# google-research/hyperbo

Measured on AMD Instinct MI355X. Metric: GP NLL+grad evals/sec at N=8192 D=16 fp64, higher is better.
Workload: dtype f64

## Files before the change

### hyperbo_amd/csrc/chol.hip

```cpp
#include "hbo_internal.h"
#include <type_traits>
#include <limits.h>
#include <string.h>

namespace {

#include "panel_dev.h"
#ifdef HBO_POTF2_TIMING
__device__ unsigned long long hbo_dbg_stamps[64];
__device__ unsigned long long hbo_dbg_wall[3 * 256];
__device__ unsigned long long hbo_dbg_trsm[3 * 128];
__device__ int hbo_dbg_trsm_panel = 36;
#define STAMP(i) do { if (threadIdx.x == 0) hbo_dbg_stamps[i] = __builtin_readcyclecounter(); } while (0)
#else
#define STAMP(i) do {} while (0)
#endif
#ifndef HBO_POTF2_WAVES
#define HBO_POTF2_WAVES 8
#endif
constexpr int POTF2_WAVES = HBO_POTF2_WAVES;
constexpr int POTF2_THREADS = 64 * POTF2_WAVES;
template <typename T>
__device__ __forceinline__ void potf2_body(const TaskDesc& t, int p, int* info_slot, unsigned char* smem) {
  typedef typename Mma<T>::acc_t acc_t;
// ... 71 lines not shown

  int nleaf = 8;
  {
    const int64_t rows = (int64_t)t.n - (int64_t)p * NB;
    if (rows < NB) nleaf = rows <= 0 ? 0 : (int)((rows + 15) / 16);
    for (int jb = nleaf + wave; jb < 8; jb += POTF2_WAVES)
#pragma unroll
      for (int r = 0; r < 4; ++r) {
        const int row = Mma<T>::crow(lane, r);
        gst(Wb + (int64_t)(jb * 16 + row) * ld + jb * 16 + l15, row == l15 ? (T)1 : (T)0);
      }
    if (tid < NB && tid >= nleaf * 16) sDinv[tid] = (T)1;
  }
  const bool lead_tile0 = nleaf > 0;
  acc_t tile0 = {0, 0, 0, 0};
  if (wave == 0 && lead_tile0) {
#pragma unroll
    for (int r = 0; r < 4; ++r) {
      const int row = Mma<T>::crow(lane, r);
      const int rr = row > l15 ? row : l15, cc = row > l15 ? l15 : row;
      tile0[r] = gld(Ab + (int64_t)rr * ld + cc);
    }
  }
  constexpr int NSH = POTF2_THREADS / 256;
  const int sh = __builtin_amdgcn_readfirstlane(tid >> 8);
  T vload[36 / NSH];
  auto load_issue = [&](auto share) {
    constexpr int SH = decltype(share)::value;
    int tile = 0;
#pragma unroll
    for (int I = 0; I < 8; ++I)
#pragma unroll
      for (int J = 0; J <= I; ++J, ++tile) {
        if (tile % NSH != SH) continue;
        if (tile == 0 && lead_tile0) { vload[0] = (T)0; continue; }
        int r = ei, c = ej;
        if (I == J && ej > ei) { r = ej; c = ei; }
        vload[tile / NSH] = gld(Ab + (int64_t)(I * 16 + r) * ld + J * 16 + c);
      }
  };
  auto load_commit = [&](auto share) {
    constexpr int SH = decltype(share)::value;
#pragma unroll
    for (int k = 0; k < 36 / NSH; ++k)
      if (!(k == 0 && SH == 0 && lead_tile0)) sT[(k * NSH + SH) * TILE_ELEMS + ei * TS + ej] = vload[k];
  };
  static_assert(NSH == 1 || NSH == 2, "one or two 256-thread groups");
  if (NSH == 1 || sh == 0) load_issue(std::integral_constant<int, 0>());
  else load_issue(std::integral_constant<int, NSH - 1>());
  if (wave == 0 && lead_tile0) factor_leaf(0, &tile0);
  if (NSH == 1 || sh == 0) load_commit(std::integral_constant<int, 0>());
  else load_commit(std::integral_constant<int, NSH - 1>());
  STAMP(1);
  __syncthreads();
  STAMP(2);
  for (int jb = 0; jb < nleaf; ++jb) {
    for (int R = jb + 1 + wave; R < nleaf; R += POTF2_WAVES) solve_tile(jb, R);
    __syncthreads();
    STAMP(3 + 3 * jb);
    if (jb == nleaf - 1) break;
    {
      const int m = nleaf - 1 - jb;
      const int ntiles = m * (m + 1) / 2;
      constexpr int NH = POTF2_WAVES == 8 ? 6 : POTF2_WAVES - 1;
      const int hw = POTF2_WAVES == 8 ? (wave < 4 ? wave : wave - 1) : wave;
      const int n0 = (ntiles - 1 > 4 * NH + 1) ? (ntiles - 1 - (4 * NH + 1)) / POTF2_WAVES : 0;
      const int nshared = ntiles - n0;
      auto tile_of = [&](int tix, int& I, int& J) {
        int ii = 0;
        while ((ii + 1) * (ii + 2) / 2 <= tix) ++ii;
        I = jb + 1 + ii; J = jb + 1 + tix - ii * (ii + 1) / 2;
      };
      if (wave == 0) {
        update_tile(jb, jb + 1, jb + 1);
        factor_leaf(jb + 1);
        STAMP(4 + 3 * jb);
        for (int tix = nshared; tix < ntiles; ++tix) { int I, J; tile_of(tix, I, J); update_tile(jb, I, J); }
      } else if (!(POTF2_WAVES == 8 && wave == 4)) {
        int tix = hw;
        for (; tix + NH < nshared; tix += 2 * NH) {
          int I0, J0, I1, J1;
          tile_of(tix, I0, J0); tile_of(tix + NH, I1, J1);
          update_tile2(jb, I0, J0, I1, J1);
        }
        if (tix < nshared) { int I, J; tile_of(tix, I, J); update_tile(jb, I, J); }
      }
    }
    __syncthreads();
    STAMP(5 + 3 * jb);
  }
  STAMP(30);

  auto store_share = [&](auto share) {
    constexpr int SH = decltype(share)::value;
    int tile = 0;
#pragma unroll
    for (int I = 0; I < 8; ++I)
#pragma unroll
      for (int J = 0; J <= I; ++J, ++tile) {
        if (tile % NSH != SH) continue;
        T v = sT[tile * TILE_ELEMS + ei * TS + ej];
        if (I == J && ej > ei) v = (T)0;
        gst(Ab + (int64_t)(I * 16 + ei) * ld + J * 16 + ej, v);
      }
  };
  if (NSH == 1 || sh == 0) store_share(std::integral_constant<int, 0>());
// ... 222 lines not shown
```

### hyperbo_amd/csrc/gram.hip

```cpp
#include "kernfun.h"

namespace {

template <typename T, bool PADDED, int KID>
__global__ __launch_bounds__(256) void gram_kernel(GramArgs g, const ModelDev* __restrict__ md) {
  typedef typename V16<T>::type vec_t;
  constexpr int VEC = 16 / sizeof(T);
  __shared__ T sA[DC * SXS];
  __shared__ T sB[DC * SXS];
  const int ti = blockIdx.y;
  const int tj = g.symmetric ? (int)((blockIdx.x + blockIdx.y) % gridDim.x) : (int)blockIdx.x;
  const T* x1; const T* x2; T* out; int64_t n1, n2, ldo; int64_t e1, e2;
  if (g.tasks) {
    const TaskDesc& t = g.tasks[blockIdx.z];
    md += (int64_t)blockIdx.z * g.model_stride;
    if ((int64_t)ti * GTR >= t.npad || tj >= t.nblk) return;
    x1 = x2 = static_cast<const T*>(t.F);
    out = static_cast<T*>(t.A);
    n1 = n2 = t.n; ldo = t.ld; e1 = e2 = t.npad;
  } else {
    x1 = static_cast<const T*>(g.x1); x2 = static_cast<const T*>(g.x2); out = static_cast<T*>(g.out);
    n1 = g.n1; n2 = g.n2; ldo = g.ldo; e1 = PADDED ? g.n1pad : g.n1; e2 = PADDED ? g.n2pad : g.n2;
  }
  const int64_t r0 = (int64_t)ti * GTR, c0 = (int64_t)tj * HBO_TILE;
  if (g.symmetric && c0 > r0 + GTR - 1) return;
  const int fdim = g.fdim;
  constexpr int kid = KID;
  constexpr bool is_dot = (kid == HBO_KERNEL_DOT);
  const int tid = threadIdx.x, tx = tid & 15, ty = tid >> 4;

  T acc[GRA][8];
#pragma unroll
  for (int a = 0; a < GRA; ++a)
#pragma unroll
    for (int b = 0; b < 8; ++b) acc[a][b] = (T)0;

  for (int d0 = 0; d0 < fdim; d0 += DC) {
    __syncthreads();
    stage_x<T, GRA>(sA, x1, n1, fdim, r0, d0, md->inv_ls, !is_dot, tid);
    stage_x<T, 8>(sB, x2, n2, fdim, c0, d0, md->inv_ls, !is_dot, tid);
    __syncthreads();
    const int dlim = (fdim - d0) < DC ? (fdim - d0) : DC;
    auto step = [&](int dd) {
      T av[GRA], bv[8];
#pragma unroll
      for (int a = 0; a < GRA; ++a) av[a] = sA[dd * SXS + ty + 16 * a];
#pragma unroll
      for (int q = 0; q < 8; ++q) bv[q] = sB[dd * SXS + 16 * VEC * (q / VEC) + VEC * tx + (q % VEC)];
      if (is_dot) {
#pragma unroll
        for (int a = 0; a < GRA; ++a)
#pragma unroll
          for (int q = 0; q < 8; ++q) acc[a][q] += av[a] * bv[q];
      } else {
#pragma unroll
        for (int a = 0; a < GRA; ++a)
#pragma unroll
          for (int q = 0; q < 8; ++q) { const T df = av[a] - bv[q]; acc[a][q] += df * df; }
      }
    };
    for (int dd = 0; dd < dlim; ++dd) step(dd);
  }

  const ExpCoef ec = hbo_exp_coef();
// ... 18 lines not shown
          vv[e] = kfun(kid, acc[a][qb * VEC + e], sv, inv_sigma2, bias2, ec);
#endif
        }
#ifdef HBO_GRAM_NOSTORE
        if (vv[0] == (T)123.456) gst(reinterpret_cast<vec_t*>(orow + 16 * VEC * qb), vv);
#else
        gst(reinterpret_cast<vec_t*>(orow + 16 * VEC * qb), vv);
#endif
      }
    }
    return;
  }
#pragma unroll
  for (int a = 0; a < GRA; ++a) {
    __builtin_amdgcn_sched_barrier(0);
    const int64_t row = r0 + ty + 16 * a;
    if (row >= e1) continue;
#pragma unroll
    for (int qb = 0; qb < 8 / VEC; ++qb) {
      const int64_t col0 = c0 + 16 * VEC * qb + VEC * tx;
      T vals[VEC];
#pragma unroll
      for (int e = 0; e < VEC; ++e) {
        const int64_t col = col0 + e;
        T v;
        if (row < n1 && col < n2) {
#ifdef HBO_GRAM_NOEXP
          v = acc[a][qb * VEC + e] * sv;
#else
          v = kfun(kid, acc[a][qb * VEC + e], sv, inv_sigma2, bias2, ec);
#endif
          if (g.symmetric && row == col) v += diag_add;
        } else {
          v = (g.symmetric && row == col) ? (T)1 : (T)0;
        }
        vals[e] = v;
      }
      if (PADDED) {
        vec_t vv;
#pragma unroll
        for (int e = 0; e < VEC; ++e) vv[e] = vals[e];
#ifdef HBO_GRAM_NOSTORE
        if (vv[0] == (T)123.456) gst(reinterpret_cast<vec_t*>(out + row * ldo + col0), vv);
#else
        gst(reinterpret_cast<vec_t*>(out + row * ldo + col0), vv);
#endif
      } else {
#pragma unroll
        for (int e = 0; e < VEC; ++e)
          if (col0 + e < e2) gst(out + row * ldo + col0 + e, vals[e]);
      }
    }
  }
}

typedef __bf16 gm_bf16x8 __attribute__((ext_vector_type(8)));
typedef float gm_f32x16 __attribute__((ext_vector_type(16)));
typedef unsigned short gm_u16x8 __attribute__((ext_vector_type(8)));
constexpr int GM_KC = 16;
constexpr int GM_ROWB = 2 * GM_KC + 16;
constexpr int GM_LPR = GM_KC / 4;
constexpr int GM_RPP = 256 / GM_LPR;
constexpr int GM_NQ = 256 / GM_RPP;
constexpr int GM_FS = HBO_TILE + 4;
constexpr float GM_RISK = 1e-6f / (32.f * 5.9604645e-8f);
constexpr unsigned GM_REDO = 0x7fc0d1e5u;
struct GmTile {
  const float* x1; const float* x2; const float* xc; float* out; const double* inv_ls;
  int64_t n1, n2, ldo, e1, e2, r0, c0;
  int fdim, nrow, ncol;
  bool symmetric, mirror, on_diag, interior;
  float sv, diag_add, risk_lim;
};
template <int KID>
__device__ __forceinline__ float gm_cov(float sv, float u) {
  if (KID == HBO_KERNEL_SE) return sv * __builtin_amdgcn_exp2f(u * (-0.5f * 1.44269504088896341f));
  const float r = __builtin_amdgcn_sqrtf((KID == HBO_KERNEL_MATERN32 ? 3.f : 5.f) * u);
  const float e = sv * __builtin_amdgcn_exp2f(r * -1.44269504088896341f);
  return KID == HBO_KERNEL_MATERN32 ? e * (1.f + r) : e * fmaf(r, fmaf(r, 1.f / 3.f, 1.f), 1.f);
}
template <int KID, bool DIRECT>
__device__ __forceinline__ bool gm_finish(const GmTile& t, const gm_f32x16 (&acc)[2][2], const float (*sN)[128]) {
  const int lane = threadIdx.x & 63, wave = threadIdx.x >> 6;
  const int wm = wave >> 1, wn = wave & 1, l32 = lane & 31, lh = lane >> 5;
  float risk = 0.f;
#pragma unroll
  for (int b = 0; b < 2; ++b) {
    const int rl = wm * 64 + b * 32 + l32;
    const float na = sN[0][rl];
    const int64_t gr = t.r0 + rl;
    float* orow = t.out + gr * t.ldo + t.c0;
#pragma unroll
    for (int a = 0; a < 2; ++a) {
      __builtin_amdgcn_sched_barrier(0);
#pragma unroll
      for (int j = 0; j < 4; ++j) {
        const int cl = wn * 64 + a * 32 + 8 * j + 4 * lh;
        const float4 nb4 = *reinterpret_cast<const float4*>(&sN[1][cl]);
        const float nbv[4] = {nb4.x, nb4.y, nb4.z, nb4.w};
        float val[4];
#pragma unroll
        for (int e = 0; e < 4; ++e) {
          const float s = acc[a][b][4 * j + e];
          const bool self = t.on_diag && rl == cl + e;
          val[e] = gm_cov<KID>(t.sv, self ? 0.f : (DIRECT ? s : fmaxf(na + nbv[e] - 2.f * s, 0.f)));
          if (!DIRECT) risk = fmaxf(risk, self ? 0.f : val[e] * (na + nbv[e]));
// ... 19 lines not shown
          }
        }
      }
    }
  }
  return risk > t.risk_lim;
}
template <int KID>
__device__ __forceinline__ void gm_direct_tile(const GmTile t, float* sF, const float (*sN)[128]) {
  const int tid = threadIdx.x, lane = tid & 63, wave = tid >> 6;
  const int wm = wave >> 1, wn = wave & 1, l32 = lane & 31, lh = lane >> 5;
  gm_f32x16 acc[2][2];
#pragma unroll
  for (int a = 0; a < 2; ++a)
#pragma unroll
    for (int b = 0; b < 2; ++b)
#pragma unroll
      for (int q = 0; q < 16; ++q) acc[a][b][q] = 0.f;
  for (int d0 = 0; d0 < t.fdim; d0 += GM_KC) {
    __syncthreads();
#pragma nounroll
    for (int i = tid; i < 2 * GM_KC * HBO_TILE; i += 256) {
      const int opq = i / (GM_KC * HBO_TILE), k = (i / HBO_TILE) % GM_KC, rr = i % HBO_TILE, d = d0 + k;
      const int64_t gr = (opq ? t.c0 : t.r0) + rr;
      float sx = 0.f;
      if (d < t.fdim && gr < (opq ? t.n2 : t.n1)) sx = ((opq ? t.x2 : t.x1)[gr * t.fdim + d] - t.xc[d]) * (float)t.inv_ls[d];
      sF[(opq * GM_KC + k) * GM_FS + rr] = sx;
    }
    __syncthreads();
#pragma nounroll
    for (int k = 0; k < GM_KC; ++k) {
      const float* fr = sF + k * GM_FS;
      const float* fc = sF + (GM_KC + k) * GM_FS;
#pragma unroll
      for (int b = 0; b < 2; ++b) {
        const float ra = fr[wm * 64 + b * 32 + l32];
#pragma unroll
        for (int a = 0; a < 2; ++a)
#pragma unroll
          for (int j = 0; j < 4; ++j) {
            const float4 cb = *reinterpret_cast<const float4*>(fc + wn * 64 + a * 32 + 8 * j + 4 * lh);
            const float cv[4] = {cb.x, cb.y, cb.z, cb.w};
#pragma unroll
            for (int e = 0; e < 4; ++e) { const float df = ra - cv[e]; acc[a][b][4 * j + e] = fmaf(df, df, acc[a][b][4 * j + e]); }
          }
      }
    }
  }
  gm_finish<KID, true>(t, acc, sN);
}
template <int KID>
__device__ __forceinline__ bool gm_make_tile(const GramArgs& g, const ModelDev*& md, GmTile& t) {
  const int ti = blockIdx.y;
  const int tj = g.symmetric ? (int)((blockIdx.x + blockIdx.y) % gridDim.x) : (int)blockIdx.x;
  if (g.tasks) {
    const TaskDesc& k = g.tasks[blockIdx.z];
    md += (int64_t)blockIdx.z * g.model_stride;
    if (ti >= k.nblk || tj >= k.nblk) return false;
    t.x1 = t.x2 = static_cast<const float*>(k.F);
    t.out = static_cast<float*>(k.A);
    t.n1 = t.n2 = k.n; t.ldo = k.ld; t.e1 = t.e2 = k.npad;
  } else {
    t.x1 = static_cast<const float*>(g.x1); t.x2 = static_cast<const float*>(g.x2); t.out = static_cast<float*>(g.out);
    t.n1 = g.n1; t.n2 = g.n2; t.ldo = g.ldo; t.e1 = g.padded ? g.n1pad : g.n1; t.e2 = g.padded ? g.n2pad : g.n2;
  }
  t.mirror = !g.tasks && !g.symmetric && t.x1 == t.x2 && t.n1 == t.n2;
  t.symmetric = g.symmetric;
  t.r0 = (int64_t)ti * HBO_TILE; t.c0 = (int64_t)tj * HBO_TILE;
  if ((g.symmetric || t.mirror) && tj > ti) return false;
  if (t.r0 >= t.e1 || t.c0 >= t.e2 || t.n1 <= 0) return false;
  t.fdim = g.fdim;
  t.xc = t.x1 + (t.r0 < t.n1 ? t.r0 : t.n1 - 1) * (int64_t)t.fdim;
  t.inv_ls = md->inv_ls;
  t.nrow = (int)min(t.n1 - t.r0, (int64_t)HBO_TILE); t.ncol = (int)min(t.n2 - t.c0, (int64_t)HBO_TILE);
  t.on_diag = (g.symmetric || t.mirror) && ti == tj;
  return true;
}
template <int KID>
__device__ __forceinline__ void gm_epilogue_fields(const ModelDev* md, GmTile& t) {
  t.interior = t.r0 + HBO_TILE <= t.n1 && t.c0 + HBO_TILE <= t.n2 && !t.on_diag && !t.mirror && (t.ldo & 3) == 0 &&
               (reinterpret_cast<unsigned long long>(t.out) & 15) == 0;
  t.sv = (float)md->sv; t.diag_add = (float)(md->noise + md->eps);
  constexpr float kappa = KID == HBO_KERNEL_SE ? 0.5f : (KID == HBO_KERNEL_MATERN32 ? 1.5f : 5.f / 6.f);
  t.risk_lim = (GM_RISK / kappa) * t.sv;
}
template <int KID>
__global__ __launch_bounds__(256, 3) void gram_mfma_kernel(GramArgs g, const ModelDev* __restrict__ md0) {
  __shared__ __attribute__((aligned(16))) unsigned char sP[2 * 3 * 128 * GM_ROWB];
  __shared__ float sN[2][128];
  GmTile t;
  const ModelDev* md = md0;
  if (!gm_make_tile<KID>(g, md, t)) return;
  const float* x1 = t.x1; const float* x2 = t.x2; const float* xc = t.xc; const double* inv_ls = t.inv_ls;
  const int64_t n1 = t.n1, n2 = t.n2, r0 = t.r0, c0 = t.c0;
  const int fdim = t.fdim;
  const int tid = threadIdx.x, lane = tid & 63, wave = tid >> 6;
  const int wm = wave >> 1, wn = wave & 1, l32 = lane & 31, lh = lane >> 5;

  const int sc4 = tid % GM_LPR, srow = tid / GM_LPR;
  const bool vec_ok = (fdim & 3) == 0 && ((reinterpret_cast<unsigned long long>(x1) | reinterpret_cast<unsigned long long>(x2)) & 15) == 0;
  auto load4 = [&](const float* xr, int d) -> float4 {
    if (vec_ok && d + 4 <= fdim) return *reinterpret_cast<const float4*>(xr + d);
    return make_float4(d < fdim ? xr[d] : 0.f, d + 1 < fdim ? xr[d + 1] : 0.f, d + 2 < fdim ? xr[d + 2] : 0.f, d + 3 < fdim ? xr[d + 3] : 0.f);
  };
  auto load_chunk = [&](int d0, float4 (&v)[GM_NQ]) {
    const int d = d0 + 4 * sc4;
#pragma unroll
// ... 409 lines not shown
```

### hyperbo_amd/csrc/hbo_internal.h

```cpp
#pragma once
#include <hip/hip_runtime.h>
#include <stdint.h>
#include "../../include/hbo.h"

#define HBO_GLOBAL __attribute__((address_space(1)))
template <typename V> __device__ __forceinline__ V gld(const V* p) { return *(const HBO_GLOBAL V*)(p); }
template <typename V> __device__ __forceinline__ void gst(V* p, V v) { *(HBO_GLOBAL V*)(p) = v; }

#define HBO_TILE 128
#define HBO_N_COUNTERS 4096
#define HBO_N_BULK_COUNTERS 1024
#define HBO_LEAF 16

struct TaskDesc {
  void* A;
  void* W;
  void* S;
  void* wscr;
  const void* X;
  const void* F;
  const void* Fm;
  const void* ysum;
  void* svec;
  void* dF;
// ... 112 lines not shown
  h = __builtin_bit_cast(unsigned short, hh); l = __builtin_bit_cast(unsigned short, ll);
}
__device__ __forceinline__ float hbo_h2_scale_for(float amax) {
  if (!(amax > 0.f) || !(amax < INFINITY)) return 1.f;
  int e;
  (void)frexpf(amax, &e);
  e = e < -40 ? -40 : e;
  return ldexpf(1.f, 14 - e);
}
__device__ __forceinline__ int yield_enter(int* tab) {
  const int tok = cu_token();
  __hip_atomic_fetch_add(tab + tok, 1, __ATOMIC_RELAXED, __HIP_MEMORY_SCOPE_AGENT);
  return tok;
}
__device__ __forceinline__ void yield_leave(int* tab, int tok) {
  __hip_atomic_fetch_add(tab + tok, -1, __ATOMIC_RELAXED, __HIP_MEMORY_SCOPE_AGENT);
}
__device__ __forceinline__ void tl_begin(unsigned long long* tl) {
#ifdef HBO_TIMELINE
  if (tl && threadIdx.x == 0) atomicMin(tl, (unsigned long long)wall_clock64());
#endif
}
__device__ __forceinline__ void tl_end(unsigned long long* tl) {
#ifdef HBO_TIMELINE
  if (tl && threadIdx.x == 0) atomicMax(tl + 1, (unsigned long long)wall_clock64());
#endif
}
#endif

static inline bool hbo_first_use_on_device(unsigned long long& seen) {
  int d = 0;
  if (hipGetDevice(&d) != hipSuccess || d < 0 || d >= 64) return true;
  if ((seen >> d) & 1ull) return false;
  seen |= 1ull << d;
  return true;
}

void launch_gemm(int dtype, const GemmArgs& a, dim3 grid, hipStream_t st);

void launch_potf2(int dtype, const TaskDesc* tasks, int ntasks, int p, int* info, hipStream_t st, int* yield_flag = nullptr,
                  unsigned long long* tl = nullptr);
void launch_trsm(int dtype, const TaskDesc* tasks, int ntasks, int p, int max_nblk, hipStream_t st, int* yield_tab = nullptr,
                 unsigned long long* tl = nullptr);
unsigned long long* tl_slot(const char* name, int p);
void launch_trtri_diag(int dtype, const TaskDesc* tasks, int ntasks, int p_lo, int p_hi, hipStream_t st);

struct GramArgs {
  const TaskDesc* tasks;
  const void* x1; const void* x2; void* out;
  int64_t n1, n2, ldo;
  int n1pad, n2pad;
  int fdim;
  int symmetric;
  int padded;
  int kernel_id;
  int direct_form;
  int mfma_min_f;
  int model_stride;
};
void launch_gram(int dtype, const GramArgs& a, const ModelDev* model, dim3 grid, hipStream_t st);
void launch_kdiag(int dtype, const void* f, int64_t n, int fdim, const ModelDev* model, void* out,
                  hipStream_t st);
void launch_dense_tanh(int dtype, const void* in, const void* w, const void* b, void* out, int64_t n,
                       int fin, int fout, hipStream_t st);
void launch_mean(int dtype, const void* fm, int64_t n, int fmean, const ModelDev* model, void* mu,
                 hipStream_t st);
void launch_aug_rows(int dtype, const TaskDesc* tasks, int ntasks, int max_npad, const ModelDev* md, hipStream_t st, int model_stride = 0);
void launch_poison(int dtype, const TaskDesc* tasks, int ntasks, int max_npad, hipStream_t st);
void launch_nll_reduce(int dtype, const TaskDesc* tasks, int ntasks, const int* info, double* out,
                       hipStream_t st);
void launch_wt_z(int dtype, const TaskDesc* tasks, int ntasks, int max_nblk, int aug_row, int out_col,
                 int out_ld, hipStream_t st, const void* xover = nullptr, void* oover = nullptr);
int grad_nacc(int kernel_id, int fdim);
void launch_grad_contract(int dtype, const TaskDesc* tasks, int ntasks, int max_nblk, const ModelDev* md,
                          int kernel_id, int fdim, int obj, double* partials, int64_t stride_task, hipStream_t st);
void launch_dmu(int dtype, const TaskDesc* tasks, int ntasks, int obj, hipStream_t st);
void launch_grad_finalize(int dtype, const TaskDesc* tasks, int ntasks, const ModelDev* md, int kernel_id,
                          int fdim, int obj, const double* partials, int64_t stride_task, double* out,
                          int out_stride, double* value_out, hipStream_t st, double* pre = nullptr, int max_nblk = 0);
constexpr int HBO_GRAD_PRE_ROWS = 32;
void launch_scale_dF(const TaskDesc* tasks, int ntasks, int64_t max_n, int fdim, hipStream_t st);
void launch_grad_feat(int dtype, const TaskDesc* tasks, int ntasks, int max_nblk, const ModelDev* md, int kernel_id,
                      int fdim, int obj, hipStream_t st);
void launch_grad_feat_mean(int dtype, const TaskDesc* tasks, int ntasks, int64_t max_n, const ModelDev* md,
                           int fdim, hipStream_t st);
void launch_dense_bwd(int dtype, const void* in, const void* out, const void* w, double* dout, double* din,
                      double* dW, double* db, int64_t n, int fin, int fout, hipStream_t st);
int small_eval_lds(int dtype);
void launch_small_eval(int dtype, const TaskDesc* tasks, int ntasks, const ModelDev* md, int kernel_id, int fdim, int* info,
                       double* nll_out, double* grad_out, int out_stride, int write_back, hipStream_t st, int tasks_per_model = 0);
struct MlpTaskDev {
  const void* x;
  void* acts[HBO_MAX_MLP_LAYERS];
  double* dF; double* dtmp;
  int64_t n;
  int64_t model;
};
void launch_mlp_forward_batch(int dtype, const MlpTaskDev* mt, int ntasks, int64_t max_n, int layer, const void* w, const void* b, int fin,
                              int fout, hipStream_t st, int model_weights = 0);
void launch_mlp_zero_dF_batch(const MlpTaskDev* mt, int ntasks, int64_t max_n, int flast, hipStream_t st);
void launch_dense_bwd_batch(int dtype, const MlpTaskDev* mt, int ntasks, int64_t max_n, int layer, int cur_is_dF, const void* w, double* dW,
                            double* db, int fin, int fout, int want_din, hipStream_t st);
void launch_kumar_forward(int dtype, const TaskDesc* tasks, int ntasks, int64_t max_n, const void* x, void* w, double* h, int64_t n, int D,
                          const ModelDev* md, hipStream_t st);
void launch_kumar_grad(int dtype, const TaskDesc* tasks, int ntasks, int max_nblk, const ModelDev* md, int kernel_id, int D, int obj,
                       double* partials, double* out, hipStream_t st);
void launch_kumar_chain_dx(int dtype, const void* xq, int64_t M, int D, const ModelDev* md, const double* gf, double* gx, hipStream_t st);
struct PostArgs {
  const void* Kxq; int64_t ldq; int npad; int n; int nblk;
  const void* alpha;
  const void* colsq;
// ... 109 lines not shown
```

### hyperbo_amd/csrc/objective.hip

```cpp
#include "api_internal.h"
#include <chrono>

extern "C" int hbo_nll(hbo_ctx* c, const hbo_model* m, hbo_dataset* ds, double* nll_sum, double* nll_per_task,
                       double* grad_sum) {
  return hbo_objective(c, m, ds, HBO_OBJ_NLL, nll_sum, nll_per_task, grad_sum);
}

int comm_allreduce_device(hbo_ctx* c, double* d_buf, int count, hipStream_t st);

int comm_abort(hbo_ctx* c);

static void enqueue_mlp_forward(hbo_ctx* c, const hbo_model* m, hbo_dataset* ds, int64_t max_n) {
  int fin = m->input_dim;
  for (int l = 0; l < m->n_layers; ++l) {
    launch_mlp_forward_batch(ds->dtype, ds->d_mlp, ds->ntasks, max_n, l, c->d_mlp_w[l], c->d_mlp_b[l], fin, m->features[l], c->stream);
    fin = m->features[l];
  }
}
static void enqueue_kumar_forward(hbo_ctx* c, const hbo_model* m, hbo_dataset* ds, int64_t max_n) {
  launch_kumar_forward(ds->dtype, ds->d_desc, ds->ntasks, max_n, nullptr, nullptr, nullptr, 0, m->input_dim, c->d_model, c->stream);
}
void enqueue_fused_forward(hbo_ctx* c, const hbo_model* m, hbo_dataset* ds, int64_t max_n, int out_stride, bool want_grad) {
  const bool kumar = is_kumar(m);
  if (needs_mlp(m)) { ProfScope ps(c, "features", 1); enqueue_mlp_forward(c, m, ds, max_n); }
// ... 146 lines not shown
    }
    if (!ds->d_mlp) HIPCHK(c, dev_alloc(c, (void**)&ds->d_mlp, sizeof(MlpTaskDev) * T));
    if (ds->h_mlp_dev.size() != (size_t)T || memcmp(ds->h_mlp_dev.data(), hm.data(), sizeof(MlpTaskDev) * T) != 0) {
      HIPCHK(c, hipStreamSynchronize(st));
      ds->h_mlp_dev = hm;
      HIPCHK(c, hipMemcpyAsync(ds->d_mlp, ds->h_mlp_dev.data(), sizeof(MlpTaskDev) * T, hipMemcpyHostToDevice, st));
    }
  }
  if (!ds->d_desc) HIPCHK(c, dev_alloc(c, (void**)&ds->d_desc, sizeof(TaskDesc) * T));
  const int out_stride = (m->kernel_id == HBO_KERNEL_DOT ? 0 : m->n_lengthscale) + 6 + mean_feature_dim(m);
  const size_t pack_bytes = sizeof(double) * T * (1 + (size_t)out_stride) + sizeof(int) * T;
  if (ds->pack_bytes < pack_bytes) {
    if (ds->d_pack) dev_free(c, ds->d_pack);
    ds->d_pack = nullptr; ds->pack_bytes = 0;
    HIPCHK(c, dev_alloc(c, (void**)&ds->d_pack, pack_bytes));
    ds->pack_bytes = pack_bytes;
  }
  ds->d_nll = ds->d_pack; ds->d_gradout = ds->d_pack + T; ds->d_info = reinterpret_cast<int*>(ds->d_pack + T + (size_t)T * out_stride);
  unsigned char* stage = static_cast<unsigned char*>(pinned_stage(c, std::max(sizeof(TaskDesc) * T, pack_bytes)));
  if (!stage) return fail(c, HBO_ERR_HIP, "hbo_objective: pinned staging buffer");
  if (ds->h_desc_dev.size() != (size_t)T || memcmp(ds->h_desc_dev.data(), ds->h_desc.data(), sizeof(TaskDesc) * T) != 0) {
    HIPCHK(c, hipEventSynchronize(c->ev_upload));
    memcpy(stage, ds->h_desc.data(), sizeof(TaskDesc) * T);
    HIPCHK(c, hipMemcpyAsync(ds->d_desc, stage, sizeof(TaskDesc) * T, hipMemcpyHostToDevice, st));
    HIPCHK(c, hipEventRecord(c->ev_upload, st));
    ds->h_desc_dev = ds->h_desc;
  }
  if (!(obj == OBJ_NLL && ds->max_nblk == 1 && small_ok)) HIPCHK(c, hipMemsetD32Async(reinterpret_cast<hipDeviceptr_t>(ds->d_info), INT_MAX, T, st));

  const int max_nblk = ds->max_nblk, max_npad = max_nblk * HBO_TILE;
  const bool fused_small = obj == OBJ_NLL && max_nblk == 1 && small_ok;
  auto mlp_forward = [&]() { enqueue_mlp_forward(c, m, ds, max_n); };
  auto kumar_forward = [&]() { enqueue_kumar_forward(c, m, ds, max_n); };
  if (fused_small) {
    enqueue_fused_forward(c, m, ds, max_n, out_stride, want_grad);
  } else {
  if (c->opt_poison) launch_poison(dtype, ds->d_desc, T, max_npad, st);
  {
    ProfScope ps(c, "features", 1);
    if (needs_mlp(m)) mlp_forward();
    launch_aug_rows(dtype, ds->d_desc, T, max_npad, c->d_model, st);
  }
  if (kumar) { ProfScope ps(c, "kumar_forward", 1); kumar_forward(); }
  int max_naug = 1;
  for (int k = 0; k < T; ++k) max_naug = std::max(max_naug, ds->h_desc[k].naug);
  TrtriProgress trtri_pg;
  SweepState sweep_st;
  hipStream_t side = st; hipEvent_t ev_side = nullptr;
  const bool la = use_lookahead(c, T, max_nblk);
  const bool sweep = want_grad && !euc && use_sweep(c, dtype, T, max_nblk);
  if (sweep) sweep_st.qs = c->opt_sweep_qs > 0 ? c->opt_sweep_qs : sweep_group(T, max_nblk);
  const bool early_trtri = !sweep && want_grad && use_early_trtri(c, T, max_nblk);
  if (!euc) {
    {
      ProfScope ps(c, "gram", 1);
      GramArgs g = {}; g.kernel_id = c->h_model->kernel_id; g.mfma_min_f = c->opt_gram_mfma; g.tasks = ds->d_desc; g.fdim = feature_dim(m); g.symmetric = 1; g.padded = 1;
      launch_gram(dtype, g, c->d_model, dim3(max_nblk, max_nblk, T), st);
    }
    {
      c->trtri_host_task = TaskDesc{};
      if (T == 1) c->trtri_host_task = ds->h_desc[0];
      c->run.chol_diag_bound = chol_diag_bound_of(m);
      ProfScope ps(c, "potrf", 1); run_potrf(c, dtype, ds->d_desc, T, max_nblk, ds->d_info, early_trtri ? &trtri_pg : nullptr, sweep ? &sweep_st : nullptr);
    }
    side = (want_grad && obj == OBJ_NLL && la) ? c->stream2 : st;
    if (side != st) { hipEvent_t e = pool_event(c, 2); hipEventRecord(e, st); hipStreamWaitEvent(side, e, 0); }
    { ProfScope ps(c, "nll_reduce", 1, side); launch_nll_reduce(dtype, ds->d_desc, T, ds->d_info, ds->d_nll, side); }
  }

  auto extra_rows = [&]() -> int {
    size_t zbytes = 0;
    if (!euc) for (int k = 0; k < T; ++k) if (ds->h_desc[k].nvec) zbytes = std::max(zbytes, (size_t)ds->tasks[k]->m * ds->tasks[k]->npad * esize(dtype));
    void* const zb = zbytes ? ws_get(c, WS_EXTRA_Z, zbytes) : nullptr;
    if (zbytes && !zb) return HBO_ERR_HIP;
    for (int k = 0; k < T; ++k) {
      if (!ds->h_desc[k].nvec) continue;
      TaskHost* t = ds->tasks[k];
      const size_t es = esize(dtype);
      char* cols = static_cast<char*>(t->svec) + (size_t)t->npad * es;
      launch_expand_rows(dtype, t->ydiv, t->n, t->npad, cols, t->m, st);
      if (euc) continue;
      launch_tri_matvec(dtype, t->W, t->ld, t->npad, cols, t->npad, t->m, 0, zb, t->npad, st);
      launch_add_sumsq(dtype, zb, t->npad, t->m, ds->h_desc[k].coef_c, ds->d_nll + k, st);
      launch_tri_matvec(dtype, t->W, t->ld, t->npad, zb, t->npad, t->m, 1, cols, t->npad, st);
    }
    return HBO_OK;
  };
  if (extras && !euc && !want_grad) {
    { ProfScope ps(c, "trtri", 1); run_trtri(c, dtype, ds->d_desc, T, max_nblk, &trtri_pg); }
    ProfScope ps(c, "extra_rows", 1);
    rc = extra_rows(); if (rc) return rc;
  }
  const int fdim = feature_dim(m);
  const int nacc = grad_nacc(m->kernel_id, fdim);
  const int64_t stride_task = (int64_t)(max_nblk * (max_nblk + 1)) * nacc;
  if (want_grad || euc) {
    const size_t pb = sizeof(double) * (stride_task * T + (size_t)HBO_GRAD_PRE_ROWS * nacc * T);
    if (ds->partials_bytes < pb) { if (ds->d_partials) dev_free(c, ds->d_partials); HIPCHK(c, dev_alloc(c, (void**)&ds->d_partials, pb)); ds->partials_bytes = pb; }
    if (!euc && sweep) {
      hipEvent_t e = side != st ? pool_event(c, 3) : nullptr;
      { ProfScope ps(c, "sweep_tail", 1);
        sweep_advance(c, dtype, ds->d_desc, T, max_nblk, max_nblk, st, sweep_st, e); }
      if (side != st) hipStreamWaitEvent(side, e, 0);
      { ProfScope ps(c, "wt_z", 1, side);
        for (int b = 0; b < max_naug; ++b) launch_wt_z(dtype, ds->d_desc, T, max_nblk, b, b, max_npad, side); }
      if (side != st) {
        launch_dmu(dtype, ds->d_desc, T, obj, side);
        ev_side = pool_event(c, 4); hipEventRecord(ev_side, side);
        hipStreamWaitEvent(st, ev_side, 0);
      }
    } else if (!euc) {
      { ProfScope ps(c, "trtri", 1);
        run_trtri(c, dtype, ds->d_desc, T, max_nblk, &trtri_pg); }
      if (side != st) { hipEvent_t e = pool_event(c, 3); hipEventRecord(e, st); hipStreamWaitEvent(side, e, 0); }
      { ProfScope ps(c, "wt_z", 1, side);
        for (int b = 0; b < max_naug; ++b) launch_wt_z(dtype, ds->d_desc, T, max_nblk, b, b, max_npad, side); }
// ... 179 lines not shown
```

### hyperbo_amd/csrc/sched.h

```cpp
#pragma once
#include "runtime.h"

struct TrtriProgress { int diag = 0; int a[12] = {0}; int b[12] = {0}; };

struct SweepState {
  int qs = 4; int done = 0; TrtriProgress pg;
  int nev = 0;
  hipEvent_t ev_c = nullptr, ev_d = nullptr;
  hipStream_t st_c = nullptr, st_d = nullptr;
};
int sweep_group(int ntasks, int max_nblk);

hipEvent_t pool_event(hbo_ctx* c, size_t i);
static inline bool use_lookahead(const hbo_ctx* c, int ntasks, int max_nblk) {
  if (!c->opt_lookahead || max_nblk <= 1) return false;
  if (c->opt_lookahead >= 2) return true;
  return max_nblk > 4 && (max_nblk >= 18 || (int64_t)ntasks * max_nblk >= 80);
}
static inline bool use_early_trtri(const hbo_ctx* c, int ntasks, int max_nblk) {
  return use_lookahead(c, ntasks, max_nblk) && c->opt_overlap_trtri && max_nblk >= 4;
}
enum YieldMode { YIELD_NONE, YIELD_POTF2, YIELD_CHAIN };
enum Fp32Form { FORM_MFMA, FORM_BF16X3, FORM_F16X2 };
struct PotrfPlan {
  bool la;
  int q, q_inner;
  int persist_free;
  int tgran, early_at;
  YieldMode yield;
  bool split_f1;
  Fp32Form form;
  bool h2_scales;
};
PotrfPlan potrf_plan(const hbo_ctx* c, int dtype, int ntasks, int max_nblk, bool sweep);
void run_potrf(hbo_ctx* c, int dtype, const TaskDesc* d_tasks, int ntasks, int max_nblk, int* d_info, TrtriProgress* early = nullptr,
               SweepState* sweep = nullptr);
bool use_sweep(const hbo_ctx* c, int dtype, int ntasks, int max_nblk);
void sweep_advance(hbo_ctx* c, int dtype, const TaskDesc* d_tasks, int ntasks, int max_nblk, int cfin, hipStream_t st, SweepState& sw,
                   hipEvent_t w_done = nullptr);
void trtri_advance(hbo_ctx* c, int dtype, const TaskDesc* d_tasks, int ntasks, int max_nblk, int cfin, hipStream_t st, TrtriProgress& pg,
                   int max_s = 1 << 30);
void run_trtri(hbo_ctx* c, int dtype, const TaskDesc* d_tasks, int ntasks, int max_nblk, TrtriProgress* pg = nullptr);
void run_lauum(hbo_ctx* c, int dtype, const TaskDesc* d_tasks, int ntasks, int max_nblk, hipStream_t st = nullptr);
```

### hyperbo_amd/csrc/sched.hip

```cpp
#include "sched.h"

#include <algorithm>
#include <cmath>

#ifdef HBO_TIMELINE
namespace {
constexpr int TL_MAX = 16384;
unsigned long long* g_tl_dev = nullptr;
int g_tl_n = 0;
bool g_tl_on = false;
struct TlEntry { char name[16]; int p; };
TlEntry g_tl_entries[TL_MAX];
}
unsigned long long* tl_slot(const char* name, int p) {
  if (!g_tl_on || g_tl_n >= TL_MAX) return nullptr;
  strncpy(g_tl_entries[g_tl_n].name, name, 15); g_tl_entries[g_tl_n].name[15] = 0;
  g_tl_entries[g_tl_n].p = p;
  return g_tl_dev + 2 * g_tl_n++;
}
extern "C" int hbo_dbg_timeline(int begin, unsigned long long* times, char* names, int* ps) {
  if (begin) {
    if (!g_tl_dev && hipMalloc(reinterpret_cast<void**>(&g_tl_dev), sizeof(unsigned long long) * 2 * TL_MAX) != hipSuccess) return -1;
    static unsigned long long init[2 * TL_MAX];
    for (int i = 0; i < TL_MAX; ++i) { init[2 * i] = ~0ull; init[2 * i + 1] = 0; }
// ... 42 lines not shown
}
template <typename Args>
static void resident_grid(hbo_ctx* c, Args& a, const GridRule& r, int64_t tiles, hipStream_t st) {
  a.persistent = 0; a.work_counter = nullptr;
  if (r.beside) {
    const int pblocks = 2 * (c->n_cus - r.free_cus);
    if (tiles > pblocks && ((a.work_counter = take_counter(r.pool)) || r.static_ok)) a.persistent = pblocks;
  } else if (r.whole && tiles >= r.whole_min) {
    if ((a.work_counter = r.whole_pool ? take_counter(r.whole_pool) : post_counter(c, st)) || r.static_ok) a.persistent = 2 * (c->n_cus - r.whole_free);
  }
}

PotrfPlan potrf_plan(const hbo_ctx* c, int dtype, int ntasks, int max_nblk, bool sweep) {
  PotrfPlan pl = {};
  pl.la = use_lookahead(c, ntasks, max_nblk);
  const bool s3 = dtype == HBO_F32 && c->opt_syrk_bf16x3;
  pl.h2_scales = dtype == HBO_F32 && c->opt_chol_f16x2 && c->run.chol_diag_bound > 0;
  pl.form = (s3 && max_nblk > 1) ? (pl.h2_scales ? FORM_F16X2 : FORM_BF16X3) : FORM_MFMA;
  const bool small_mat = max_nblk <= 96;
  const bool s3_large = s3 && !small_mat;
  const int q_small = (s3 && ntasks == 1 && max_nblk >= 56) ? 6 : ((ntasks == 1 && max_nblk > 64) ? 7 : 3);
  pl.q = c->opt_group > 0 ? c->opt_group : ((!pl.la && ntasks <= 8) ? 1 : (small_mat ? q_small : (s3_large ? 16 : (max_nblk >= 256 ? 8 : 4))));
  const int q_inner = c->opt_group_inner >= 0 ? c->opt_group_inner : ((s3_large && pl.q == 16) ? 8 : 0);
  pl.q_inner = (q_inner > 0 && q_inner < pl.q) ? q_inner : 0;
  pl.persist_free = c->opt_persist_free >= 0 ? c->opt_persist_free : 32;
  pl.split_f1 = pl.la && c->stream3 && (c->opt_split_f1 >= 2 || (c->opt_split_f1 == 1 && ntasks > 1));
  pl.tgran = 4;
  pl.early_at = -1;
  if (ntasks == 1) {
    pl.early_at = c->opt_trtri_at > 0 ? std::min(c->opt_trtri_at * max_nblk / 64, max_nblk - 1) : (max_nblk * 5 / 8) & ~3;
    if (pl.early_at < 4) pl.early_at = -1;
    pl.tgran = 1 << 30;
  }
  const bool batch_yield = ntasks > 1 && sweep && batch_bg(c, ntasks) >= 2;
  const bool yield = pl.la && c->opt_cu_yield && ((ntasks == 1 && (small_mat || pl.form != FORM_MFMA)) || batch_yield);
  pl.yield = !yield ? YIELD_NONE : (c->opt_cu_yield >= 2 ? YIELD_CHAIN : YIELD_POTF2);
  return pl;
}

namespace {
struct PotrfState {
  hbo_ctx* c; int dtype; const TaskDesc* d_tasks; int ntasks, max_nblk; int* d_info;
  hipStream_t sm, sp;
  int* yield_flag = nullptr;
  int* chain_mark = nullptr;
  TileCounters bulk = {};
  Fp32Form form = FORM_MFMA;
  Syrk3Args s3a = {};
  unsigned short* s3buf[2] = {nullptr, nullptr};
  float* h2_aug = nullptr;
  size_t evi = 0;
  hipEvent_t ev_f1b = nullptr;
  hipEvent_t ev_f2 = nullptr;
};
int tiles_of(const PotrfState& s, int c_lo, int c_hi) { int n = 0; for (int cc = c_lo; cc < std::min(c_hi, s.max_nblk); ++cc) n += s.max_nblk + 1 - cc; return n; }
void wait_f1b(PotrfState& s) { if (s.ev_f1b) { hipStreamWaitEvent(s.sp, s.ev_f1b, 0); s.ev_f1b = nullptr; } }

void potrf_setup(const PotrfPlan& pl, PotrfState& s) {
  hbo_ctx* c = s.c;
  s.yield_flag = pl.yield != YIELD_NONE ? c->d_yield : nullptr;
  if (s.yield_flag) hipMemsetAsync(s.yield_flag, 0, sizeof(int) * HBO_YIELD_TAB_ENTRIES, s.sm);
  s.chain_mark = pl.yield == YIELD_CHAIN ? s.yield_flag : nullptr;
  c->run.gemm_yield = s.yield_flag;
  int* counters = (int*)ws_get(c, WS_COUNTERS, sizeof(int) * HBO_N_COUNTERS);
  if (counters) hipMemsetAsync(counters, 0, sizeof(int) * HBO_N_COUNTERS, s.sm);
  s.bulk = {counters, 0, HBO_N_BULK_COUNTERS};
  c->run.side = {counters ? counters + HBO_N_BULK_COUNTERS : nullptr, 0, HBO_N_COUNTERS - HBO_N_BULK_COUNTERS - 512};
  c->run.post_counter_next = 0;
  s.form = pl.form;
  if (s.form != FORM_MFMA) {
    s.s3a.tasks = s.d_tasks; s.s3a.nkb = pl.q * (HBO_TILE / 16);
    s.s3a.task_stride = (int64_t)(s.max_nblk + 1) * s.s3a.nkb * 3 * (HBO_TILE * 16);
    const size_t bytes = sizeof(unsigned short) * (size_t)s.s3a.task_stride * s.ntasks;
    s.s3buf[0] = static_cast<unsigned short*>(ws_get(c, WS_SYRK3_A, bytes));
    s.s3buf[1] = static_cast<unsigned short*>(ws_get(c, WS_SYRK3_B, bytes));
    if (!s.s3buf[0] || !s.s3buf[1]) s.form = FORM_MFMA;
  }
  c->run.h2_words = nullptr;
  if (pl.h2_scales) {
    c->run.h2_words = static_cast<unsigned int*>(ws_get(c, WS_H2_SCALES, sizeof(unsigned int) * HBO_H2_WORDS));
    if (c->run.h2_words) hipMemsetAsync(c->run.h2_words, 0, sizeof(unsigned int) * HBO_H2_WORDS, s.sm);
  }
  if (s.form == FORM_F16X2) {
    s.form = FORM_BF16X3;
    if (c->run.h2_words) {
      s.s3a.aug_stride = (int64_t)(s.s3a.nkb / 4) * 8;
      s.h2_aug = static_cast<float*>(ws_get(c, WS_H2_AUG, sizeof(float) * 2 * (size_t)s.s3a.aug_stride * s.ntasks));
      if (s.h2_aug) { s.form = FORM_F16X2; s.s3a.h2 = 1; s.s3a.sx = s.s3a.sy = post2h_scale_for(std::sqrt(c->run.chol_diag_bound)); }
    }
  }
}

void step_inner_update(const PotrfPlan& pl, PotrfState& s, int g0, int g1, int gi, int p) {
  hbo_ctx* c = s.c;
  const int qi = pl.q_inner;
  if (s.form != FORM_MFMA) {
    ProfScope ps(c, "split3", 2, s.sp);
    Syrk3Args a = s.s3a; a.kcol0 = (gi - qi) * HBO_TILE; a.nk_split = qi * (HBO_TILE / 16); a.r_lo = gi; a.kb_off = (gi - qi - g0) * (HBO_TILE / 16);
    launch_split3_panel(a, s.max_nblk + 1 - gi, s.ntasks, s.sp);
  }
  wait_f1b(s);
  ProfScope ps(c, "syrk_inner", 2, s.sp);
  if (s.form != FORM_MFMA) {
    Syrk3Args a = s.s3a; a.kb_off = (gi - qi - g0) * (HBO_TILE / 16); a.nk = qi * (HBO_TILE / 16); a.c_lo = gi; a.c_hi = g1;
    a.yield_mark = s.chain_mark;
    launch_syrk3(a, tiles_of(s, gi, g1), s.ntasks, s.sp);
  } else {
    GemmArgs a = {}; a.tasks = s.d_tasks; a.mode = GEMM_SYRK; a.p0 = gi - qi; a.kt = qi; a.c_lo = gi; a.c_hi = g1; a.aug = 1;
    a.small_tiles = (int64_t)(s.max_nblk + 1 - gi) * (g1 - gi) * s.ntasks < 600;
    a.yield_mark = s.chain_mark; a.tl = tl_slot("syrk_inner", p);
    launch_gemm(s.dtype, a, dim3(s.max_nblk + 1 - gi, g1 - gi, s.ntasks), s.sp);
  }
}
void step_column_update(PotrfState& s, int gi, int p) {
  wait_f1b(s);
  ProfScope ps(s.c, "syrk_col", 2, s.sp);
  GemmArgs a = {}; a.tasks = s.d_tasks; a.mode = GEMM_SYRK; a.p0 = gi; a.kt = p - gi; a.c_lo = p; a.c_hi = p + 1; a.aug = 1; a.small_tiles = 1;
  a.yield_mark = s.chain_mark; a.tl = tl_slot("syrk_col", p);
  launch_gemm(s.dtype, a, dim3(s.max_nblk + 1 - p, 1, s.ntasks), s.sp);
}
void step_panel(PotrfState& s, int g0, int g1, int gi, int p) {
  hbo_ctx* c = s.c;
  { ProfScope ps(c, "potf2", 2, s.sp); launch_potf2(s.dtype, s.d_tasks, s.ntasks, p, s.d_info, s.sp, s.yield_flag, tl_slot("potf2", p)); }
  { ProfScope ps(c, "trsm", 2, s.sp); launch_trsm(s.dtype, s.d_tasks, s.ntasks, p, s.max_nblk, s.sp, s.chain_mark, tl_slot("trsm", p)); }
  if (s.form != FORM_MFMA && p + 1 == g1 && p + 1 < s.max_nblk) {
    ProfScope ps(c, "split3", 2, s.sp);
    Syrk3Args a = s.s3a; a.kcol0 = gi * HBO_TILE; a.nk_split = (p + 1 - gi) * (HBO_TILE / 16); a.r_lo = p + 1; a.kb_off = (gi - g0) * (HBO_TILE / 16);
    launch_split3_panel(a, s.max_nblk + 1 - (p + 1), s.ntasks, s.sp);
  }
}
void step_hand_over(const PotrfPlan& pl, PotrfState& s, int p, TrtriProgress* early, SweepState* sweep) {
  hbo_ctx* c = s.c;
  if (p + 1 >= s.max_nblk) return;
  const bool to_sweep = sweep && (p + 1) % sweep->qs == 0;
  if (!to_sweep && !(early && ((p + 1) % pl.tgran == 0 || p + 1 == pl.early_at))) return;
  hipEvent_t e = pool_event(c, s.evi++);
  hipEventRecord(e, s.sp);
  hipStreamWaitEvent(c->stream4, e, 0);
  if (to_sweep) {
    ProfScope ps(c, "sweep_early", 1, c->stream4);
    sweep_advance(c, s.dtype, s.d_tasks, s.ntasks, s.max_nblk, p + 1, c->stream4, *sweep);
  } else {
    ProfScope ps(c, "trtri_early", 1, c->stream4);
    trtri_advance(c, s.dtype, s.d_tasks, s.ntasks, s.max_nblk, p + 1, c->stream4, *early);
  }
}
void step_f1(const PotrfPlan& pl, PotrfState& s, int g0, int g1, int g2) {
  hbo_ctx* c = s.c;
  GemmArgs a = {}; a.tasks = s.d_tasks; a.mode = GEMM_SYRK; a.p0 = g0; a.kt = g1 - g0; a.aug = 1;
  a.yield_flag = s.chain_mark ? nullptr : s.yield_flag;
  a.yield_mark = s.chain_mark;
  if (s.ev_f2) hipStreamWaitEvent(s.sp, s.ev_f2, 0);
  wait_f1b(s);
  ProfScope ps(c, "syrk_trailing", 1, s.sp);
  a.c_lo = g1; a.c_hi = pl.la ? g2 : s.max_nblk;
  if (s.form != FORM_MFMA) {
    Syrk3Args b = s.s3a; b.kb_off = 0; b.nk = (g1 - g0) * (HBO_TILE / 16); b.c_lo = a.c_lo; b.c_hi = a.c_hi;
    b.yield_mark = a.yield_mark; b.yield_flag = a.yield_flag;
    launch_syrk3(b, tiles_of(s, b.c_lo, b.c_hi), s.ntasks, s.sp);
    return;
  }
  if (pl.split_f1 && a.c_hi - a.c_lo > 1) {
    hipEvent_t e = pool_event(c, s.evi++);
    hipEventRecord(e, s.sp); hipStreamWaitEvent(c->stream3, e, 0);
    GemmArgs b = a; b.c_lo = a.c_lo + 1;
    b.small_tiles = (int64_t)(s.max_nblk + 1 - b.c_lo) * (b.c_hi - b.c_lo) * s.ntasks < 600;
    b.tl = tl_slot("f1b", g1);
    launch_gemm(s.dtype, b, dim3(s.max_nblk + 1 - b.c_lo, b.c_hi - b.c_lo, s.ntasks), c->stream3);
    s.ev_f1b = pool_event(c, s.evi++);
    hipEventRecord(s.ev_f1b, c->stream3);
    a.c_hi = a.c_lo + 1;
  }
  a.small_tiles = (int64_t)(s.max_nblk + 1 - a.c_lo) * (a.c_hi - a.c_lo) * s.ntasks < 600;
  a.tl = tl_slot("f1", g1);
  launch_gemm(s.dtype, a, dim3(s.max_nblk + 1 - a.c_lo, a.c_hi - a.c_lo, s.ntasks), s.sp);
}
void step_f2(const PotrfPlan& pl, PotrfState& s, int g0, int g1, int g2) {
  hbo_ctx* c = s.c;
  const int64_t m = s.max_nblk - g2;
  const bool small_tiles = m * (m + 1) / 2 * s.ntasks < 600;
  const int nt = tiles_of(s, g2, s.max_nblk);
  {
    ProfScope ps(c, small_tiles ? "syrk_trailing" : "syrk_bulk", 1, s.sm);
    GridRule r; r.pool = &s.bulk;
    if (s.form != FORM_MFMA) {
      Syrk3Args b = s.s3a; b.kb_off = 0; b.nk = (g1 - g0) * (HBO_TILE / 16); b.c_lo = g2; b.c_hi = s.max_nblk;
      r.beside = s.ntasks == 1 && c->opt_syrk3_free > 0; r.free_cus = c->opt_syrk3_free;
      resident_grid(c, b, r, nt, s.sm);
      b.yield_flag = s.yield_flag;
      launch_syrk3(b, nt, s.ntasks, s.sm);
    } else {
      GemmArgs a = {}; a.tasks = s.d_tasks; a.mode = GEMM_SYRK; a.p0 = g0; a.kt = g1 - g0; a.aug = 1;
      a.yield_flag = s.yield_flag;
      a.c_lo = g2; a.c_hi = s.max_nblk; a.small_tiles = small_tiles;
      const int pblocks = 2 * (c->n_cus - pl.persist_free);
      const int64_t ntiles = (int64_t)nt * (small_tiles ? 4 : 1);
      r.beside = s.ntasks == 1 && pl.persist_free > 0 && m <= 96; r.free_cus = pl.persist_free;
      r.whole = s.ntasks == 1 && pl.persist_free > 0 && m > 96 && c->opt_lauum_persist && !small_tiles; r.whole_pool = &s.bulk;
      r.static_ok = true;
      resident_grid(c, a, r, ntiles, s.sm);
      if (a.persistent && a.work_counter && !small_tiles) {
        const int64_t rem = ntiles % pblocks;
        if (rem > 0 && rem * 2 <= pblocks) a.n_big = (int)(ntiles - rem);
      }
      a.tl = tl_slot("f2", g1);
      launch_gemm(s.dtype, a, dim3(s.max_nblk + 1 - a.c_lo, a.c_hi - a.c_lo, s.ntasks), s.sm);
    }
  }
  s.ev_f2 = pool_event(c, s.evi++);
  hipEventRecord(s.ev_f2, s.sm);
}
}

void run_potrf(hbo_ctx* c, int dtype, const TaskDesc* d_tasks, int ntasks, int max_nblk, int* d_info, TrtriProgress* early,
               SweepState* sweep) {
  const PotrfPlan pl = potrf_plan(c, dtype, ntasks, max_nblk, sweep != nullptr);
  PotrfState s = {c, dtype, d_tasks, ntasks, max_nblk, d_info, c->stream, pl.la ? c->stream2 : c->stream};
  if (pl.la) { hipEvent_t e = pool_event(c, s.evi++); hipEventRecord(e, s.sm); hipStreamWaitEvent(s.sp, e, 0); }
  potrf_setup(pl, s);
  c->last_chol_form = (int)s.form; c->last_inv_forms = 0;
  for (int g0 = 0, grp = 0; g0 < max_nblk; g0 += pl.q, ++grp) {
    const int g1 = std::min(g0 + pl.q, max_nblk);
    const int g2 = std::min(g1 + pl.q, max_nblk);
    if (s.form != FORM_MFMA) s.s3a.Xp = s.s3buf[grp & 1];
    if (s.form == FORM_F16X2) s.s3a.aug_scale = s.h2_aug + (grp & 1) * s.s3a.aug_stride * ntasks;
    for (int p = g0; p < g1; ++p) {
      const int gi = pl.q_inner ? g0 + (p - g0) / pl.q_inner * pl.q_inner : g0;
      if (pl.q_inner && p == gi && p > g0) step_inner_update(pl, s, g0, g1, gi, p);
      if (p > gi) step_column_update(s, gi, p);
      step_panel(s, g0, g1, gi, p);
      step_hand_over(pl, s, p, early, sweep);
    }
    if (g1 == max_nblk) break;
    step_f1(pl, s, g0, g1, g2);
    if (!pl.la) continue;
    hipEvent_t e = pool_event(c, s.evi++);
    hipEventRecord(e, s.sp); hipStreamWaitEvent(s.sm, e, 0);
    if (g2 < max_nblk) step_f2(pl, s, g0, g1, g2);
  }
  c->run.gemm_yield = nullptr;
  c->run.side.base = nullptr;
  wait_f1b(s);
  if (pl.la) { hipEvent_t e = pool_event(c, s.evi++); hipEventRecord(e, s.sp); hipStreamWaitEvent(s.sm, e, 0); }
  if (early && !sweep) {
    hipEvent_t e = pool_event(c, s.evi++);
    hipEventRecord(e, c->stream4);
    hipStreamWaitEvent(s.sm, e, 0);
  }
}
static bool trtri_level3(hbo_ctx* c, const TaskDesc* d_tasks, const TaskDesc& h, int max_nblk, int s, int grp_lo, int grp_hi,
                         bool do_a, bool do_b, hipStream_t st) {
  int ngrp = grp_hi - grp_lo;
  int vlast = std::min(s, max_nblk - ((grp_hi - 1) * 2 * s + s));
  if (vlast <= 0) { --ngrp; vlast = s; }
  if (ngrp <= 0) return true;
  const int nkb = 8 * s;
  int li = 0;
  while ((1 << li) < s) ++li;
  unsigned int* const words = (c->run.h2_words && li < HBO_H2_LEVELS) ? c->run.h2_words + 3 * li : nullptr;
  const bool h2 = words != nullptr;
  const float sL = h2 ? post2h_scale_for(std::sqrt(c->run.chol_diag_bound)) : 1.f;
  const int64_t gstride = (int64_t)s * nkb * (h2 ? 2 : 3) * (HBO_TILE * 16);
  const size_t bytes = sizeof(unsigned short) * (size_t)gstride * ngrp;
  unsigned short* xp = static_cast<unsigned short*>(ws_get(c, WS_TRTRI3_X, bytes));
  unsigned short* yp = static_cast<unsigned short*>(ws_get(c, WS_TRTRI3_Y, bytes));
  if (!xp || !yp) return false;
  const int64_t ld = h.ld;
  const int64_t o0 = (int64_t)grp_lo * 2 * s * HBO_TILE, half = (int64_t)s * HBO_TILE;
  const float* L = static_cast<const float*>(h.A);
  const float* W = static_cast<const float*>(h.W);
  const float* S = static_cast<const float*>(h.S);
  Split3Block sb = {}; sb.ld = ld; sb.gstep = 2 * half * (ld + 1); sb.gstride = gstride; sb.nkb = nkb; sb.row_tiles = s;
// ... 197 lines not shown
```

Baseline: 93.93.

## Split gram build so first panel columns start Cholesky before rest finishes

The symmetric gram kernel now takes a column offset. For single-task lookahead runs it is launched in two parts: the first q block-columns go on the main stream, and the remaining columns are launched on the main stream inside run_potrf after potrf setup, with an event recorded after them. The panel stream, which must first wait on the main stream, can then start factoring the first group while the rest of the matrix is still being generated, and the early trtri/sweep stream and the first trailing SYRK wait on that event. The aim is to overlap gram construction with the first panel factorizations, at the cost of an extra launch and more cross-stream event dependencies that must be correct. Timeline hooks and a debug timestamp are also added.

```diff
diff --git a/hyperbo_amd/csrc/chol.hip b/hyperbo_amd/csrc/chol.hip
--- a/hyperbo_amd/csrc/chol.hip
+++ b/hyperbo_amd/csrc/chol.hip
@@ -147,6 +147,9 @@
   if (NSH == 1 || sh == 0) load_commit(std::integral_constant<int, 0>());
   else load_commit(std::integral_constant<int, NSH - 1>());
   STAMP(1);
+#ifdef HBO_POTF2_TIMING
+  if (tid == 64) hbo_dbg_stamps[33] = __builtin_readcyclecounter();
+#endif
   __syncthreads();
   STAMP(2);
   for (int jb = 0; jb < nleaf; ++jb) {
diff --git a/hyperbo_amd/csrc/gram.hip b/hyperbo_amd/csrc/gram.hip
--- a/hyperbo_amd/csrc/gram.hip
+++ b/hyperbo_amd/csrc/gram.hip
@@ -8,8 +8,9 @@
   constexpr int VEC = 16 / sizeof(T);
   __shared__ T sA[DC * SXS];
   __shared__ T sB[DC * SXS];
+  tl_begin(g.tl);
   const int ti = blockIdx.y;
-  const int tj = g.symmetric ? (int)((blockIdx.x + blockIdx.y) % gridDim.x) : (int)blockIdx.x;
+  const int tj = g.symmetric ? g.col0 + (int)((blockIdx.x + blockIdx.y) % gridDim.x) : (int)blockIdx.x;
   const T* x1; const T* x2; T* out; int64_t n1, n2, ldo; int64_t e1, e2;
   if (g.tasks) {
     const TaskDesc& t = g.tasks[blockIdx.z];
@@ -134,6 +135,7 @@
       }
     }
   }
+  tl_end(g.tl);
 }
 
 typedef __bf16 gm_bf16x8 __attribute__((ext_vector_type(8)));
@@ -259,7 +261,7 @@
 template <int KID>
 __device__ __forceinline__ bool gm_make_tile(const GramArgs& g, const ModelDev*& md, GmTile& t) {
   const int ti = blockIdx.y;
-  const int tj = g.symmetric ? (int)((blockIdx.x + blockIdx.y) % gridDim.x) : (int)blockIdx.x;
+  const int tj = g.symmetric ? g.col0 + (int)((blockIdx.x + blockIdx.y) % gridDim.x) : (int)blockIdx.x;
   if (g.tasks) {
     const TaskDesc& k = g.tasks[blockIdx.z];
     md += (int64_t)blockIdx.z * g.model_stride;
diff --git a/hyperbo_amd/csrc/hbo_internal.h b/hyperbo_amd/csrc/hbo_internal.h
--- a/hyperbo_amd/csrc/hbo_internal.h
+++ b/hyperbo_amd/csrc/hbo_internal.h
@@ -188,11 +188,13 @@
   int n1pad, n2pad;
   int fdim;
   int symmetric;
+  int col0;
   int padded;
   int kernel_id;
   int direct_form;
   int mfma_min_f;
   int model_stride;
+  unsigned long long* tl;
 };
 void launch_gram(int dtype, const GramArgs& a, const ModelDev* model, dim3 grid, hipStream_t st);
 void launch_kdiag(int dtype, const void* f, int64_t n, int fdim, const ModelDev* model, void* out,
diff --git a/hyperbo_amd/csrc/objective.hip b/hyperbo_amd/csrc/objective.hip
--- a/hyperbo_amd/csrc/objective.hip
+++ b/hyperbo_amd/csrc/objective.hip
@@ -222,16 +222,31 @@
   if (sweep) sweep_st.qs = c->opt_sweep_qs > 0 ? c->opt_sweep_qs : sweep_group(T, max_nblk);
   const bool early_trtri = !sweep && want_grad && use_early_trtri(c, T, max_nblk);
   if (!euc) {
+    std::function<void(hipStream_t)> gram_rest;
     {
       ProfScope ps(c, "gram", 1);
       GramArgs g = {}; g.kernel_id = c->h_model->kernel_id; g.mfma_min_f = c->opt_gram_mfma; g.tasks = ds->d_desc; g.fdim = feature_dim(m); g.symmetric = 1; g.padded = 1;
-      launch_gram(dtype, g, c->d_model, dim3(max_nblk, max_nblk, T), st);
+      const int q = (la && T == 1) ? potrf_plan(c, dtype, T, max_nblk, sweep).q : 0;
+      if (q > 0 && q < max_nblk) {
+        g.tl = tl_slot("gram", 0);
+        launch_gram(dtype, g, c->d_model, dim3(q, max_nblk, T), st);
+        g.col0 = q;
+        gram_rest = [c, dtype, g, max_nblk, q](hipStream_t s2) mutable {
+          ProfScope ps(c, "gram", 1, s2);
+          g.tl = tl_slot("gram", q);
+          launch_gram(dtype, g, c->d_model, dim3(max_nblk - q, max_nblk, 1), s2);
+        };
+      } else {
+        g.tl = tl_slot("gram", 0);
+        launch_gram(dtype, g, c->d_model, dim3(max_nblk, max_nblk, T), st);
+      }
     }
     {
       c->trtri_host_task = TaskDesc{};
       if (T == 1) c->trtri_host_task = ds->h_desc[0];
       c->run.chol_diag_bound = chol_diag_bound_of(m);
-      ProfScope ps(c, "potrf", 1); run_potrf(c, dtype, ds->d_desc, T, max_nblk, ds->d_info, early_trtri ? &trtri_pg : nullptr, sweep ? &sweep_st : nullptr);
+      ProfScope ps(c, "potrf", 1);
+      run_potrf(c, dtype, ds->d_desc, T, max_nblk, ds->d_info, early_trtri ? &trtri_pg : nullptr, sweep ? &sweep_st : nullptr, gram_rest ? &gram_rest : nullptr);
     }
     side = (want_grad && obj == OBJ_NLL && la) ? c->stream2 : st;
     if (side != st) { hipEvent_t e = pool_event(c, 2); hipEventRecord(e, st); hipStreamWaitEvent(side, e, 0); }
diff --git a/hyperbo_amd/csrc/sched.h b/hyperbo_amd/csrc/sched.h
--- a/hyperbo_amd/csrc/sched.h
+++ b/hyperbo_amd/csrc/sched.h
@@ -1,5 +1,6 @@
 #pragma once
 #include "runtime.h"
+#include <functional>
 
 struct TrtriProgress { int diag = 0; int a[12] = {0}; int b[12] = {0}; };
 
@@ -34,7 +35,7 @@
 };
 PotrfPlan potrf_plan(const hbo_ctx* c, int dtype, int ntasks, int max_nblk, bool sweep);
 void run_potrf(hbo_ctx* c, int dtype, const TaskDesc* d_tasks, int ntasks, int max_nblk, int* d_info, TrtriProgress* early = nullptr,
-               SweepState* sweep = nullptr);
+               SweepState* sweep = nullptr, const std::function<void(hipStream_t)>* rest = nullptr);
 bool use_sweep(const hbo_ctx* c, int dtype, int ntasks, int max_nblk);
 void sweep_advance(hbo_ctx* c, int dtype, const TaskDesc* d_tasks, int ntasks, int max_nblk, int cfin, hipStream_t st, SweepState& sw,
                    hipEvent_t w_done = nullptr);
diff --git a/hyperbo_amd/csrc/sched.hip b/hyperbo_amd/csrc/sched.hip
--- a/hyperbo_amd/csrc/sched.hip
+++ b/hyperbo_amd/csrc/sched.hip
@@ -118,6 +118,7 @@
   size_t evi = 0;
   hipEvent_t ev_f1b = nullptr;
   hipEvent_t ev_f2 = nullptr;
+  hipEvent_t ev_rest = nullptr;
 };
 int tiles_of(const PotrfState& s, int c_lo, int c_hi) { int n = 0; for (int cc = c_lo; cc < std::min(c_hi, s.max_nblk); ++cc) n += s.max_nblk + 1 - cc; return n; }
 void wait_f1b(PotrfState& s) { if (s.ev_f1b) { hipStreamWaitEvent(s.sp, s.ev_f1b, 0); s.ev_f1b = nullptr; } }
@@ -203,6 +204,7 @@
   hipEvent_t e = pool_event(c, s.evi++);
   hipEventRecord(e, s.sp);
   hipStreamWaitEvent(c->stream4, e, 0);
+  if (s.ev_rest) hipStreamWaitEvent(c->stream4, s.ev_rest, 0);
   if (to_sweep) {
     ProfScope ps(c, "sweep_early", 1, c->stream4);
     sweep_advance(c, s.dtype, s.d_tasks, s.ntasks, s.max_nblk, p + 1, c->stream4, *sweep);
@@ -217,6 +219,7 @@
   a.yield_flag = s.chain_mark ? nullptr : s.yield_flag;
   a.yield_mark = s.chain_mark;
   if (s.ev_f2) hipStreamWaitEvent(s.sp, s.ev_f2, 0);
+  s.ev_rest = nullptr;
   wait_f1b(s);
   ProfScope ps(c, "syrk_trailing", 1, s.sp);
   a.c_lo = g1; a.c_hi = pl.la ? g2 : s.max_nblk;
@@ -279,11 +282,15 @@
 }
 
 void run_potrf(hbo_ctx* c, int dtype, const TaskDesc* d_tasks, int ntasks, int max_nblk, int* d_info, TrtriProgress* early,
-               SweepState* sweep) {
+               SweepState* sweep, const std::function<void(hipStream_t)>* rest) {
   const PotrfPlan pl = potrf_plan(c, dtype, ntasks, max_nblk, sweep != nullptr);
   PotrfState s = {c, dtype, d_tasks, ntasks, max_nblk, d_info, c->stream, pl.la ? c->stream2 : c->stream};
   if (pl.la) { hipEvent_t e = pool_event(c, s.evi++); hipEventRecord(e, s.sm); hipStreamWaitEvent(s.sp, e, 0); }
   potrf_setup(pl, s);
+  if (rest) {
+    (*rest)(s.sm);
+    if (pl.la) { s.ev_f2 = s.ev_rest = pool_event(c, s.evi++); hipEventRecord(s.ev_f2, s.sm); }
+  }
   c->last_chol_form = (int)s.form; c->last_inv_forms = 0;
   for (int g0 = 0, grp = 0; g0 < max_nblk; g0 += pl.q, ++grp) {
     const int g1 = std::min(g0 + pl.q, max_nblk);
```

New measurement: 93.54. Within noise of the previous version (-0.4%).
